# Distributed-Learning-Networking-Group/torchgpipe

Hardware: AMD Instinct MI355X
Metric: U-Net(5,64) GPipe training throughput (samples/sec) (higher is better)
Workload: dtype fp32; 1 GPU; model=U-Net(5,64), experiment=pipeline-1, global_batch=80, input=3x192x192, chunks=2, checkpoint=except_last, parallelism=pp1, transport=none, fused_cells=True, cell_streams=0, overlap_recompute=True, overlap_forward=True, graph_cells=False, hw_queues=4

## Files before the change

torchgpipe_amd/csrc/bindings.cpp:

```cpp
#include <algorithm>
#include <torch/extension.h>
#include <ATen/hip/HIPContext.h>
#include <ATen/hip/impl/HIPGuardImplMasqueradingAsCUDA.h>

#include <vector>

#include "kernels.h"

namespace tgpipe {
namespace {

hipStream_t stream_of(const at::Tensor& t) {
  return at::hip::getCurrentHIPStream(t.device().index()).stream();
}

const int64_t* rng_state(const c10::optional<at::Tensor>& rng, const at::Device& device) {
  if (!rng.has_value() || !rng->defined()) return nullptr;
  TORCH_CHECK(rng->is_cuda() && rng->device() == device && rng->scalar_type() == at::kLong &&
                  rng->is_contiguous() && rng->numel() == 2,
              "rng must be a contiguous int64 [2] (seed, offset) tensor on the op's device");
  return rng->data_ptr<int64_t>();
}

void check_f32_gpu(const at::Tensor& t, const char* name) {
// ... 160 lines not shown
  const int64_t red_channels = flip ? w.size(0) : w.size(1);
  c10::hip::HIPGuardMasqueradingAsCUDA guard(w.device());
  auto u = transform_out(
      out, {wino4_pad_reduction(red_channels), wino4_pad_output(out_channels), 36}, w);
  launch_wino4_weight(w.data_ptr<float>(), u.data_ptr<float>(), out_channels, red_channels, flip,
                      stream_of(w));
  return u;
}

at::Tensor wino4_conv(const at::Tensor& x_in, const at::Tensor& u,
                      const c10::optional<at::Tensor>& bias, int64_t out_channels,
                      int64_t variant, int64_t splits) {
  auto x = x_in.contiguous();
  check_f32_gpu(x, "x");
  check_f32_gpu(u, "u");
  TORCH_CHECK(x.dim() == 4, "x must be NCHW");
  const int64_t n = x.size(0), r = x.size(1), h = x.size(2), w = x.size(3);
  TORCH_CHECK(u.dim() == 3 && u.size(2) == 36 && u.size(0) == wino4_pad_reduction(r) &&
                  u.size(1) == wino4_pad_output(out_channels),
              "F(4x4) transformed weight does not match the input/output channels");
  TORCH_CHECK(u.device() == x.device(), "u must live on the input's device");
  TORCH_CHECK(wino4_supported(n, r, h, w, out_channels),
              "input too large for the F(4x4) kernel (needs < 1 GiB); use wino_conv");
  const float* bptr = nullptr;
  if (bias.has_value() && bias->defined()) {
    check_f32_gpu(*bias, "bias");
    TORCH_CHECK(bias->numel() == out_channels, "bias must have K elements");
    bptr = bias->data_ptr<float>();
  }
  c10::hip::HIPGuardMasqueradingAsCUDA guard(x.device());
  auto y = at::empty({n, out_channels, h, w}, x.options());
  if (y.numel() == 0) return y;
  TORCH_CHECK(variant == -1 || (variant >= 4 && variant <= 15 && variant != 11 && variant != 13) ||
                  variant == 16 || variant == 17 || variant == 18 || (variant >= 20 && variant <= 22),
              "variant must be -1, 4-10, 12, 14-18 or 20-22");
  const WinoPlan plan = wino4_plan(n, r, h, w, out_channels, static_cast<int>(variant),
                                   static_cast<int>(splits));
  at::Tensor ws;
  if (plan.workspace > 0) ws = at::empty({plan.workspace}, x.options());
  launch_wino4_conv(x.data_ptr<float>(), u.data_ptr<float>(), bptr, y.data_ptr<float>(),
                    plan.workspace > 0 ? ws.data_ptr<float>() : nullptr, n, r, h, w,
                    out_channels, plan, stream_of(x));
  return y;
}

at::Tensor wgrad_destination(const c10::optional<at::Tensor>& into, const at::Tensor& x,
                             int64_t k, int64_t c) {
  if (!into.has_value()) return at::empty({k, c, 3, 3}, x.options());
  const at::Tensor& d = *into;
  TORCH_CHECK(d.is_contiguous() && d.scalar_type() == at::kFloat && d.device() == x.device() &&
                  d.dim() == 4 && d.size(0) == k && d.size(1) == c && d.size(2) == 3 &&
                  d.size(3) == 3,
              "into must be a contiguous fp32 [K][C][3][3] tensor on x's device");
  return d;
}

at::Tensor wino_wgrad(const at::Tensor& x_in, const at::Tensor& dy_in, int64_t splits,
                      int64_t variant, const c10::optional<at::Tensor>& into) {
  auto x = x_in.contiguous();
  auto dy = dy_in.contiguous();
  check_f32_gpu(x, "x");
  check_f32_gpu(dy, "dy");
  TORCH_CHECK(x.dim() == 4 && dy.dim() == 4, "x and dy must be NCHW");
  const int64_t n = x.size(0), c = x.size(1), h = x.size(2), w = x.size(3), k = dy.size(1);
  TORCH_CHECK(dy.size(0) == n && dy.size(2) == h && dy.size(3) == w,
              "dy must be [N][K][H][W] of a 3x3/s1/p1 convolution of x");
  TORCH_CHECK(dy.device() == x.device(), "x and dy must share a device");
  TORCH_CHECK(c * h * w < (int64_t{1} << 31) && k * h * w < (int64_t{1} << 31),
// ... 103 lines not shown
  TORCH_CHECK(plan.ksteps * 16 * plan.np < (int64_t{1} << 31) &&
                  plan.mp * plan.np < (int64_t{1} << 31),
              "operands too large for the batched-GEMM kernels");
  float* pm = nullptr;
  int ipg = 0;
  if (stats.has_value() && stats->defined()) {
    check_f32_gpu(*stats, "stats");
    ipg = bg_stats_ipg(n, h, w, static_cast<int>(kind));
    const int64_t groups = (n + ipg - 1) / ipg;
    TORCH_CHECK(stats->device() == x.device() && stats->is_contiguous() &&
                    stats->numel() == 2 * groups * out_channels,
                "stats must be a contiguous [2][ceil(n / bg_stats_ipg)][K] float32 tensor");
    pm = stats->data_ptr<float>();
  }
  auto ws = at::empty({plan.workspace}, x.options());
  launch_bg_conv(x.data_ptr<float>(), a.data_ptr<float>(), bptr, y.data_ptr<float>(),
                 ws.data_ptr<float>(), n, r, h, w, out_channels, plan, stream_of(x), pm,
                 pm == nullptr ? nullptr : pm + stats->numel() / 2, ipg);
  return y;
}

int64_t bg_stats_images(int64_t n, int64_t h, int64_t w, int64_t kind) {
  return bg_stats_ipg(n, h, w, static_cast<int>(kind));
}

int64_t wino4_splits(int64_t n, int64_t c, int64_t k, int64_t h, int64_t w, int64_t variant) {
  if (variant == 0) {
    const int64_t steps = (n * ((h + 3) / 4) * ((w + 3) / 4) + 3) / 4;
    return std::min<int64_t>(wino4_wgrad_splits(n, c, k, h, w), steps);
  }
  return wino4_plan(n, c, h, w, k, static_cast<int>(variant), 0).splits;
}

}
}

TORCH_LIBRARY(tgpipe, m) {
  m.def("dna_forward(Tensor x, float p, float eps, float slope, int seed, int offset, "
        "bool dropout, Tensor? rng=None) -> Tensor[]");
  m.def("dna_backward(Tensor dy, Tensor x, Tensor mean, Tensor rstd, Tensor scale, "
        "float slope) -> Tensor");
  m.def("dropout(Tensor x, float p, int seed, int offset, Tensor? rng=None) -> Tensor");
  m.def("philox_uniform(int n, int seed, int offset, Device device, Tensor? rng=None) -> Tensor");
  m.def("spin(int ns, Device device) -> ()");
  m.def("copy_segments(Tensor[] srcs, Tensor(a!)[] dsts) -> ()");
  m.def("wino_weight(Tensor w, bool flip, Tensor? out=None) -> Tensor");
  m.def("wino_wgrad(Tensor x, Tensor dy, int splits=0, int variant=-1, Tensor? into=None) -> Tensor");
  m.def("wino_conv(Tensor x, Tensor u, Tensor? bias, int out_channels, int variant=-1, "
        "int splits=0) -> Tensor");
  m.def("wino4_weight(Tensor w, bool flip, Tensor? out=None) -> Tensor");
  m.def("wino4_wgrad(Tensor x, Tensor dy, int splits=0, int variant=0, Tensor? into=None) -> Tensor");
  m.def("wino4_conv(Tensor x, Tensor u, Tensor? bias, int out_channels, int variant=-1, "
        "int splits=0) -> Tensor");
  m.def("bg_weight(Tensor w, bool flip, int kind=4, Tensor? out=None, int emu=-1) -> Tensor");
  m.def("wino4_splits(int n, int c, int k, int h, int w, int variant) -> int",
        &tgpipe::wino4_splits);
  m.def("bg_conv(Tensor x, Tensor a, Tensor? bias, int out_channels, int bn=0, int splits=0, "
        "int kind=4, int waves=0, int sub=0, int emu=-1, Tensor(b!)? stats=None) -> Tensor");
  m.def("bg_stats_images(int n, int h, int w, int kind) -> int", &tgpipe::bg_stats_images);
}

TORCH_LIBRARY_IMPL(tgpipe, CUDA, m) {
  m.impl("dna_forward", &tgpipe::dna_forward);
  m.impl("dna_backward", &tgpipe::dna_backward);
  m.impl("dropout", &tgpipe::dropout);
  m.impl("copy_segments", &tgpipe::copy_segments);
  m.impl("wino_weight", &tgpipe::wino_weight);
  m.impl("wino_conv", &tgpipe::wino_conv);
  m.impl("wino_wgrad", &tgpipe::wino_wgrad);
  m.impl("wino4_weight", &tgpipe::wino4_weight);
  m.impl("wino4_conv", &tgpipe::wino4_conv);
  m.impl("wino4_wgrad", &tgpipe::wino4_wgrad);
  m.impl("bg_weight", &tgpipe::bg_weight);
  m.impl("bg_conv", &tgpipe::bg_conv);
}

TORCH_LIBRARY_IMPL(tgpipe, CompositeExplicitAutograd, m) {
  m.impl("philox_uniform", &tgpipe::philox_uniform);
  m.impl("spin", &tgpipe::spin);
}

PYBIND11_MODULE(TORCH_EXTENSION_NAME, m) {
  m.doc() = "torchgpipe_amd native HIP kernels (gfx950)";
}
```

torchgpipe_amd/csrc/kernels.h:

```cpp
#pragma once
#include <hip/hip_runtime.h>
#include <stdint.h>

#include <vector>

namespace tgpipe {

void launch_dna_forward(const float* x, float* y, float* mean, float* rstd, float* scale,
                        int64_t planes, int64_t s, float p, float eps, float slope,
                        uint64_t seed, uint64_t offset, bool dropout, const int64_t* rng,
                        hipStream_t stream);

void launch_dna_backward(const float* dy, const float* x, const float* mean, const float* rstd,
                         const float* scale, float* dx, int64_t planes, int64_t s, float slope,
                         hipStream_t stream);

void launch_dropout(const float* x, float* y, int64_t n, float p, uint64_t seed, uint64_t offset,
                    const int64_t* rng, hipStream_t stream);

void launch_philox_uniform(float* out, int64_t n, uint64_t seed, uint64_t offset,
                           const int64_t* rng, hipStream_t stream);

void launch_spin(uint64_t ns, hipStream_t stream);

struct Segment {
  const void* src;
  void* dst;
  int64_t bytes;
};
constexpr int kMaxSegments = 16;
void launch_segments_copy(const Segment* segs, int count, hipStream_t stream);

int64_t wino_pad_reduction(int64_t r);
int64_t wino_pad_output(int64_t o);
void launch_wino_weight(const float* w, float* u, int64_t out_channels, int64_t red_channels,
                        bool flip, hipStream_t stream);
struct WinoPlan {
  int variant = 0;
  int splits = 1;
  int64_t workspace = 0;
};
WinoPlan wino_plan(int64_t n, int64_t red_channels, int64_t h, int64_t w, int64_t out_channels,
                   int variant, int splits);
void launch_wino_conv(const float* x, const float* u, const float* bias, float* y, float* ws,
                      int64_t n, int64_t red_channels, int64_t h, int64_t w, int64_t out_channels,
                      const WinoPlan& plan, hipStream_t stream);

int64_t wino4_pad_reduction(int64_t r);
int64_t wino4_pad_output(int64_t o);
bool wino4_supported(int64_t n, int64_t r, int64_t h, int64_t w, int64_t o);
void launch_wino4_weight(const float* w, float* u, int64_t out_channels, int64_t red_channels,
                         bool flip, hipStream_t stream);
WinoPlan wino4_plan(int64_t n, int64_t red_channels, int64_t h, int64_t w, int64_t out_channels,
                    int variant, int splits);
void launch_wino4_conv(const float* x, const float* u, const float* bias, float* y, float* ws,
                       int64_t n, int64_t red_channels, int64_t h, int64_t w, int64_t out_channels,
                       const WinoPlan& plan, hipStream_t stream);

struct BgPlan {
  int kind = 4;
  int waves = 8;
  int bn = 64;
  int sub = 1;
  int splits = 1;
  bool emu = false;
  int64_t mp = 0, np = 0, ksteps = 0;
  int64_t workspace = 0;
};
bool bg_emu(int emu);
int bg_pick_bn(int64_t tiles, int kind, bool emu = false);
BgPlan bg_plan(int64_t n, int64_t red_channels, int64_t h, int64_t w, int64_t out_channels,
               int bn, int splits, int kind, int waves, int sub, int emu = -1);
int64_t bg_weight_numel(int64_t out_channels, int64_t red_channels, int kind, int emu = -1);
void launch_bg_weight(const float* w, float* a, int64_t out_channels, int64_t red_channels,
                      bool flip, int kind, hipStream_t stream, int emu = -1);
int bg_stats_ipg(int64_t n, int64_t h, int64_t w, int kind);
void launch_bg_conv(const float* x, const float* a, const float* bias, float* y, float* ws,
                    int64_t n, int64_t red_channels, int64_t h, int64_t w, int64_t out_channels,
                    const BgPlan& plan, hipStream_t stream, float* pm = nullptr,
                    float* pm2 = nullptr, int ipg = 0);


bool wino4_wgrad_supported(int64_t n, int64_t c, int64_t k, int64_t h, int64_t w);
int wino4_wgrad_splits(int64_t n, int64_t c, int64_t k, int64_t h, int64_t w);
int wino4_wgrad_emu_splits(int64_t n, int64_t c, int64_t k, int64_t h, int64_t w);
int64_t wino4_wgrad_emu_workspace(int64_t n, int64_t c, int64_t k, int64_t h, int64_t w,
                                  int splits);
void launch_wino4_wgrad_emu(const float* x, const float* dy, float* dw, float* ws, int64_t n,
                            int64_t c, int64_t k, int64_t h, int64_t w, int splits, bool accum,
                            hipStream_t stream);
// ... 172 lines not shown
```

torchgpipe_amd/csrc/winograd_f4.hip:

```cpp
#include <hip/hip_runtime.h>
#include <stdint.h>

#include <algorithm>
#include <cstdlib>
#include <string>
#include <type_traits>

#include "kernels.h"

namespace tgpipe {
namespace {

typedef float floatx4 __attribute__((ext_vector_type(4)));
typedef float floatx2 __attribute__((ext_vector_type(2)));

constexpr int kP = 36;
constexpr int kC = 4;
constexpr int kOPad = 64;
constexpr int kT = 32;
constexpr int kVImg = kC * kT * kP;

template <int OG>
struct F4Cfg {
  static constexpr int kO = 16 * OG;
  static constexpr int kThreads = 128 * OG;
  static constexpr int kUImg = kC * kO * kP;
  static constexpr int kBuf = kUImg + kVImg;
  static constexpr int kSlabThreads = kThreads - 128;
  static constexpr int kUVec = kUImg / 4 / kSlabThreads;
  static_assert(kUVec * 4 * kSlabThreads == kUImg, "slab waves copy the slab evenly");
};
constexpr uint32_t kBadRow = 0x80000000u;
constexpr uint32_t kBadCol = 0x40000000u;

__device__ __forceinline__ void f4_weight_tile(const float* __restrict__ w, int O, int R, int o,
                                               int r, bool flip, float (&v)[kP]) {
  float g[3][3] = {};
  if (r < R && o < O) {
// ... 209 lines not shown
      acc[4 * q + e] = __builtin_amdgcn_mfma_f32_16x16x4f32(a[q][e], b[q][e], acc[4 * q + e], 0, 0, 0);
  }
  __builtin_amdgcn_sched_group_barrier(0x100, 2 * kAhead, 0);
#pragma unroll
  for (int q = 0; q < kQ; ++q) {
    if (q + kAhead < kQ) __builtin_amdgcn_sched_group_barrier(0x100, 2, 0);
    __builtin_amdgcn_sched_group_barrier(0x008, 4, 0);
  }
}

__device__ __forceinline__ void f4_fwd_offsets(F4Patch& p, int t, int c, int P, int tpi, int TW,
                                               int R, int H, int W) {
  const bool tv = t < P;
  const int tt = tv ? t : 0;
  const int n = tt / tpi;
  const int rem = tt - n * tpi;
  const int ty = rem / TW;
  const int tx = rem - ty * TW;
  const int y0 = 4 * ty - 1, x0 = 4 * tx - 1;
  const int64_t base = (static_cast<int64_t>(n) * R + c) * H * W +
                       static_cast<int64_t>(y0) * W + x0;
#pragma unroll
  for (int i = 0; i < 6; ++i) {
    const bool ok = tv && y0 + i >= 0 && y0 + i < H;
    p.row[i] = ok ? static_cast<uint32_t>((base + static_cast<int64_t>(i) * W) * 4) : kBadRow;
  }
#pragma unroll
  for (int j = 0; j < 6; ++j) {
    const bool ok = x0 + j >= 0 && x0 + j < W;
    p.col[j] = ok ? static_cast<uint32_t>(4 * j) : kBadCol;
  }
}

__device__ __forceinline__ void f4_output_transform(const floatx4 (&acc)[kP],
                                                    float* __restrict__ ydst,
                                                    const float* __restrict__ bias, int tp,
                                                    int tpi, int TW, int H, int W, int O,
                                                    int obase) {
  const int HW = H * W;
  const int pn = tp / tpi;
  const int prem = tp - pn * tpi;
  const int pty = prem / TW;
  const int py = 4 * pty;
  const int px = 4 * (prem - pty * TW);
  const bool full = (W & 3) == 0 && py + 4 <= H;
#pragma unroll
  for (int rp = 0; rp < 2; ++rp) {
    const int o = obase + 2 * rp;
    if (o >= O) continue;
    floatx2 s[4][6];
#pragma unroll
    for (int j = 0; j < 6; ++j) {
      floatx2 m[6];
#pragma unroll
      for (int i = 0; i < 6; ++i) m[i] = floatx2{acc[i * 6 + j][2 * rp], acc[i * 6 + j][2 * rp + 1]};
      const floatx2 a = m[1] + m[2], b = m[1] - m[2], c = m[3] + m[4], d = m[3] - m[4];
      s[0][j] = m[0] + a + c;
      s[1][j] = b + 2.f * d;
      s[2][j] = a + 4.f * c;
      s[3][j] = b + 8.f * d + m[5];
    }
    const floatx2 bv{bias ? bias[o] : 0.f, bias && o + 1 < O ? bias[o + 1] : 0.f};
#pragma unroll
    for (int k = 0; k < 4; ++k) {
      const floatx2 a = s[k][1] + s[k][2], b = s[k][1] - s[k][2];
      const floatx2 c = s[k][3] + s[k][4], d = s[k][3] - s[k][4];
      const floatx2 v0 = s[k][0] + a + c + bv, v1 = b + 2.f * d + bv, v2 = a + 4.f * c + bv;
      const floatx2 v3 = b + 8.f * d + s[k][5] + bv;
#pragma unroll
      for (int e = 0; e < 2; ++e) {
        if (o + e >= O) break;
        float* yp = ydst + (static_cast<int64_t>(pn) * O + o + e) * HW +
                    static_cast<int64_t>(py) * W + px;
        const floatx4 out{v0[e], v1[e], v2[e], v3[e]};
        if (full) {
          *reinterpret_cast<floatx4*>(yp + k * W) = out;
        } else if (py + k < H) {
#pragma unroll
          for (int l = 0; l < 4; ++l)
            if (px + l < W) yp[k * W + l] = out[l];
        }
      }
    }
  }
}

typedef __attribute__((address_space(3))) void lds_void_t;
typedef __attribute__((address_space(1))) void glob_void_t;

template <typename Cfg, int kWaves>
__device__ __forceinline__ void f4_glds_slab(const float* __restrict__ src, float* dst, int sw,
                                             int lane) {
  constexpr int kPieces = Cfg::kUImg / 256;
  static_assert(kPieces % kWaves == 0, "slab waves copy the slab evenly");
#pragma unroll
  for (int i = 0; i < kPieces / kWaves; ++i) {
    const int piece = i * kWaves + sw;
    __builtin_amdgcn_global_load_lds((glob_void_t*)(src + piece * 256 + lane * 4),
                                     (lds_void_t*)(dst + piece * 256), 16, 0, 0);
  }
}

template <int OG, bool kVec, bool kGlds = false, int kAblate = 0>
__global__ __launch_bounds__(F4Cfg<OG>::kThreads, 4 / OG) void f4_conv_kernel(
    const float* __restrict__ x, const float* __restrict__ u, const float* __restrict__ bias,
    float* __restrict__ y, int R, int H, int W, int O, int Rp, int Op, int TH, int TW, int P,
    int tblocks, int oblocks, int splits, uint32_t x_bytes) {
// ... 361 lines not shown
    }
    asm volatile("s_waitcnt lgkmcnt(0)" ::: "memory");
    __builtin_amdgcn_s_barrier();
    auto step = [&](int s, int buf, floatx4 (&cur)[kPer], floatx4 (&nxt)[kPer]) {
      if constexpr (!kDeep && (kDbg & 2) == 0) load_rows(cur, min(s + 3, s_end - 1));
      if (s + 1 < s_end)
        f4_glds_slab<Cfg, kGldsWaves>(ubase + (s + 1) * slab_stride, lds + (buf ^ 1) * kBuf, sw,
                                      lane);
      if constexpr (kDeep && (kDbg & 2) == 0) load_rows(nxt, min(s + 4, s_end - 1));
      __builtin_amdgcn_sched_barrier(0);
      f4_mfma<Cfg>(acc, lds + buf * kBuf, lane, wo, wt);
      __builtin_amdgcn_sched_barrier(0);
      if constexpr ((kDbg & 4) == 0) store_rows(cur, buf ^ 1);
      if constexpr (kDeep) {
        asm volatile("s_waitcnt vmcnt(%0)" ::"n"(kPer) : "memory");
      } else {
        asm volatile("s_waitcnt vmcnt(0)" ::: "memory");
      }
      asm volatile("s_waitcnt lgkmcnt(0)" ::: "memory");
      __builtin_amdgcn_s_barrier();
    };
    floatx4 rodd[kPer];
    int s = s_begin;
    for (; s + 1 < s_end; s += 2) {
      step(s, 0, rreg, rodd);
      step(s + 1, 1, rodd, rreg);
    }
    if (s < s_end) step(s, 0, rreg, rodd);
  }

  const int tp = t0 + wt * 16 + (lane & 15);
  if (tp >= P) return;
  float* ydst = y + static_cast<int64_t>(z) * (P / tpi) * O * HW;
  f4_output_transform(acc, ydst, bias != nullptr && splits == 1 ? bias : nullptr, tp, tpi, TW,
                      H, W, O, o0 + wo * 16 + 4 * (lane >> 4));
}


__global__ __launch_bounds__(256) void f4_input_transform_kernel(
    const float* __restrict__ x, float* __restrict__ v, int R, int H, int W, int TW, int tpi,
    int P, int Rp, int64_t total, uint32_t x_bytes) {
  const int64_t idx = static_cast<int64_t>(blockIdx.x) * blockDim.x + threadIdx.x;
  if (idx >= total) return;
  const int tt = static_cast<int>(idx & 31);
  const int64_t rest = idx >> 5;
  const int c4 = static_cast<int>(rest & 3);
  const int64_t sb = rest >> 2;
  const int steps = Rp / kC;
  const int s = static_cast<int>(sb % steps);
  const int tb = static_cast<int>(sb / steps);
  const int t = tb * kT + tt;
  const int c = s * kC + c4;
  float* dst = v + idx * kP;
  F4Patch p;
  if (t >= P || c >= R) {
#pragma unroll
    for (int q = 0; q < kP / 4; ++q) reinterpret_cast<floatx4*>(dst)[q] = floatx4{0.f, 0.f, 0.f, 0.f};
    return;
  }
  const __amdgpu_buffer_rsrc_t xr =
      __builtin_amdgcn_make_buffer_rsrc(const_cast<float*>(x), static_cast<short>(0),
                                        static_cast<int>(x_bytes), 0x00020000);
  f4_fwd_offsets(p, t, c, P, tpi, TW, R, H, W);
  f4_load_patch<false>(p, xr, 0);
  f4_transform_store(p, dst);
}

template <int OG, int kAhead = 2>
// ... 1616 lines not shown
      }
#pragma unroll
      for (int l = 0; l < TILE; ++l)
        if (l < cols) ts += v[k][l];
    }
    const float tc = static_cast<float>(rows * cols);
    const float tm = ts / tc;
    float tq = 0.f;
#pragma unroll
    for (int k = 0; k < TILE; ++k) {
      if (k >= rows) break;
#pragma unroll
      for (int l = 0; l < TILE; ++l) {
        if (l < cols) {
          const float d = v[k][l] - tm;
          tq += d * d;
        }
      }
    }
    chan_merge_f(cnt, mean, m2, tc, tm, tq);
  }
#pragma unroll
  for (int off = 32; off > 0; off >>= 1) {
    const float nb = __shfl_xor(cnt, off), mb = __shfl_xor(mean, off);
    const float qb = __shfl_xor(m2, off);
    chan_merge_f(cnt, mean, m2, nb, mb, qb);
  }
  if (lane == 0) {
    pm[static_cast<int64_t>(g) * O + o] = mean;
    pm2[static_cast<int64_t>(g) * O + o] = m2;
  }
}

}

int64_t wino4_pad_reduction(int64_t r) { return (r + kC - 1) / kC * kC; }
int64_t wino4_pad_output(int64_t o) { return (o + kOPad - 1) / kOPad * kOPad; }

bool wino4_supported(int64_t n, int64_t r, int64_t h, int64_t w, int64_t o) {
  const int64_t x_bytes = n * r * h * w * 4;
  const int64_t tiles = n * ((h + 3) / 4) * ((w + 3) / 4);
  return x_bytes > 0 && x_bytes < (int64_t{1} << 30) - 64 && tiles < (int64_t{1} << 30) &&
         n * o * h * w < (int64_t{1} << 31) && o < (1 << 24);
}

void launch_wino4_weight(const float* w, float* u, int64_t out_channels, int64_t red_channels,
                         bool flip, hipStream_t stream) {
  const int64_t Op = wino4_pad_output(out_channels);
  const int64_t Rp = wino4_pad_reduction(red_channels);
  const int64_t total = Rp * Op;
  hipLaunchKernelGGL(f4_weight_kernel, dim3(static_cast<unsigned>((total + 255) / 256)), dim3(256),
                     0, stream, w, u, static_cast<int>(out_channels),
                     static_cast<int>(red_channels), static_cast<int>(Op), static_cast<int>(Rp),
                     flip);
}

WinoPlan wino4_plan(int64_t n, int64_t red_channels, int64_t h, int64_t w, int64_t out_channels,
                    int variant, int splits) {
  WinoPlan plan;
  plan.variant = (variant >= 4 && variant <= 12 && variant != 11) || variant == 14 ||
                         variant == 15 || variant == 16 || variant == 17 || variant == 18 ||
                         (variant >= 20 && variant <= 22) ? variant : 5;
  if (plan.variant == 16 && ((w & 3) != 0 || w < 8)) plan.variant = 6;
  if (plan.variant == 17 && ((w & 3) != 0 || w < 24)) plan.variant = 7;
  if (plan.variant >= 20 && plan.variant <= 22 && ((w & 3) != 0 || w < 24)) plan.variant = 6;
  const int og = plan.variant == 5 || plan.variant == 7 || plan.variant == 15 ||
                         plan.variant == 17 ? 2 : 4;
  const int64_t P = n * ((h + 3) / 4) * ((w + 3) / 4);
  const int64_t blocks = ((P + kT - 1) / kT) * ((out_channels + 16 * og - 1) / (16 * og));
  const int64_t steps = wino4_pad_reduction(red_channels) / kC;
  if (splits > 0) {
    plan.splits = static_cast<int>(std::min<int64_t>(splits, steps));
  } else {
    const int64_t cap = og == 4 ? 256 : 512;
    const double step_us = og == 4 ? 2.1 : 1.9;
    const double mb = static_cast<double>(n) * out_channels * h * w * 4 / 1e6;
    int64_t best = 1;
    double best_cost = 0;
    for (int64_t s = 1; s <= std::min<int64_t>(64, steps); ++s) {
      const int64_t rounds = (blocks * s + cap - 1) / cap;
      const double cost = rounds * ((steps + s - 1) / s) * step_us +
                          (s > 1 ? 11.6 + 0.23 * s * mb : 0.0);
      if (s == 1 || cost < best_cost) {
        best = s;
        best_cost = cost;
      }
    }
    plan.splits = static_cast<int>(best);
  }
  plan.workspace = plan.splits > 1 ? plan.splits * n * out_channels * h * w : 0;
  if (plan.variant == 14 || plan.variant == 15) {
    plan.workspace += ((P + kT - 1) / kT) * kT * wino4_pad_reduction(red_channels) * kP;
  }
  return plan;
}

void launch_wino4_conv(const float* x, const float* u, const float* bias, float* y, float* ws,
                       int64_t n, int64_t red_channels, int64_t h, int64_t w, int64_t out_channels,
                       const WinoPlan& plan, hipStream_t stream) {
  const int64_t Rp = wino4_pad_reduction(red_channels);
  const int64_t Op = wino4_pad_output(out_channels);
  const int64_t th = (h + 3) / 4, tw = (w + 3) / 4;
  const int64_t P = n * th * tw;
  const int og = plan.variant == 5 || plan.variant == 7 || plan.variant == 15 ||
                         plan.variant == 17 ? 2 : 4;
  const int tblocks = static_cast<int>((P + kT - 1) / kT);
  if (plan.variant == 18) {
    const int oblocks4 = static_cast<int>((out_channels + 63) / 64);
    const int64_t nwg4 = static_cast<int64_t>(tblocks) * oblocks4 * plan.splits;
    auto kernel = f4_conv_ring_kernel<false>;
    hipLaunchKernelGGL(kernel, dim3(static_cast<unsigned>(nwg4)), dim3(512), 0, stream, x, u,
                       bias, plan.splits > 1 ? ws : y, static_cast<int>(red_channels),
                       static_cast<int>(h), static_cast<int>(w),
                       static_cast<int>(out_channels), static_cast<int>(Rp),
                       static_cast<int>(Op), static_cast<int>(th), static_cast<int>(tw),
                       static_cast<int>(P), tblocks, oblocks4, plan.splits,
                       static_cast<uint32_t>(n * red_channels * h * w * 4));
    if (plan.splits > 1)
      launch_split_reduce(ws, bias, y, n * out_channels * h * w, h * w,
                          static_cast<int>(out_channels), plan.splits, stream);
    return;
  }
// ... 4 lines not shown
    float* vbuf = ws;
    const int64_t vtotal = static_cast<int64_t>(tblocks) * kT * Rp;
    float* split_ws = ws + vtotal * kP;
    hipLaunchKernelGGL(f4_input_transform_kernel, dim3(static_cast<unsigned>((vtotal + 255) / 256)),
                       dim3(256), 0, stream, x, vbuf, static_cast<int>(red_channels),
                       static_cast<int>(h), static_cast<int>(w), static_cast<int>(tw),
                       static_cast<int>(th * tw), static_cast<int>(P), static_cast<int>(Rp),
                       vtotal, static_cast<uint32_t>(n * red_channels * h * w * 4));
    auto gemm = og == 4 ? f4_gemm_kernel<4> : f4_gemm_kernel<2>;
    hipLaunchKernelGGL(gemm, dim3(static_cast<unsigned>(nwg)), dim3(128 * og), 0, stream, vbuf, u,
                       bias, splits > 1 ? split_ws : y, static_cast<int>(h), static_cast<int>(w),
                       static_cast<int>(out_channels), static_cast<int>(Rp), static_cast<int>(Op),
                       static_cast<int>(th), static_cast<int>(tw), static_cast<int>(P), tblocks,
                       oblocks, splits);
    if (splits > 1)
      launch_split_reduce(split_ws, bias, y, n * out_channels * h * w, h * w,
                          static_cast<int>(out_channels), splits, stream);
    return;
  }
  const bool vec = (w & 3) == 0;
  auto kernel = og == 4 ? f4_conv_kernel<4, false>
                        : (vec ? f4_conv_kernel<2, true> : f4_conv_kernel<2, false>);
  if (plan.variant == 6) kernel = f4_conv_kernel<4, false, true>;
  if (plan.variant == 8) kernel = f4_conv_kernel<4, false, true, 1>;
  if (plan.variant == 9) kernel = f4_conv_kernel<4, false, true, 2>;
  if (plan.variant == 10) kernel = f4_conv_kernel<4, false, true, 3>;
  if (plan.variant == 12) kernel = vec ? f4_conv_kernel<4, true, true> : f4_conv_kernel<4, false, true>;
  if (plan.variant == 7) kernel = vec ? f4_conv_kernel<2, true, true> : f4_conv_kernel<2, false, true>;
  if (plan.variant == 16) kernel = tw >= 6 ? f4_conv_rows_kernel<46, 3> : f4_conv_rows_kernel<66, 5>;
  if (plan.variant == 17) kernel = f4_conv_rows_kernel<46, 9, 2>;
  if (plan.variant == 20) kernel = f4_conv_rows_kernel<46, 3, 4, 8>;
  if (plan.variant == 21) kernel = f4_conv_rows_kernel<46, 3, 4, 1>;
  if (plan.variant == 22) kernel = f4_conv_rows_kernel<46, 3, 4, 7>;
  hipLaunchKernelGGL(kernel, dim3(static_cast<unsigned>(nwg)), dim3(128 * og), 0, stream,
                     x, u, bias, splits > 1 ? ws : y, static_cast<int>(red_channels),
                     static_cast<int>(h), static_cast<int>(w), static_cast<int>(out_channels),
                     static_cast<int>(Rp), static_cast<int>(Op), static_cast<int>(th),
                     static_cast<int>(tw), static_cast<int>(P), tblocks, oblocks, splits,
                     static_cast<uint32_t>(n * red_channels * h * w * 4));
  if (splits > 1) {
    launch_split_reduce(ws, bias, y, n * out_channels * h * w, h * w,
                        static_cast<int>(out_channels), splits, stream);
  }
}

bool wino4_wgrad_supported(int64_t n, int64_t c, int64_t k, int64_t h, int64_t w) {
  const int64_t lim = (int64_t{1} << 30) - 64;
  const int64_t tiles = n * ((h + 3) / 4) * ((w + 3) / 4);
  return n * c * h * w * 4 < lim && n * k * h * w * 4 < lim && n * c * h * w > 0 &&
         n * k * h * w > 0 && tiles + 64 < (int64_t{1} << 30);
}

int wino4_wgrad_splits(int64_t n, int64_t c, int64_t k, int64_t h, int64_t w) {
  const int64_t blocks = ((c + 31) / 32) * ((k + 63) / 64);
  const int64_t steps = (n * ((h + 3) / 4) * ((w + 3) / 4) + 3) / 4;
  const double mb = static_cast<double>(((c + 31) / 32) * 32) * (((k + 63) / 64) * 64) * 9 * 4 /
                    1e6;
  int best = 1;
  double best_cost = 0;
  for (int64_t s = 1; s <= std::min<int64_t>(512, steps); ++s) {
    const int64_t rounds = (blocks * s + 255) / 256;
    const double cost = rounds * ((steps + s - 1) / s) * 2.5 + (s > 1 ? 5.0 + 0.8 * s * mb : 0.0);
    if (s == 1 || cost < best_cost) {
      best = static_cast<int>(s);
      best_cost = cost;
    }
  }
// ... 341 lines not shown
```

torchgpipe_amd/ops/conv.py:

```python
import os
import threading
from typing import Any, Dict, List, Optional, Sequence, Tuple
import weakref

import torch
from torch import Tensor, nn
import torch.nn.functional as F

from torchgpipe_amd.ops import _ext, gradacc

__all__ = ['WinogradConv2d', 'winograd_conv2d', 'wino_eligible', 'new_step',
           'clear_winograd_caches', 'cache_bytes', 'refresh_step_caches', 'hold_cache',
           'size_cache_budget', 'conv_with_bn_stats']

_STEP = 0
_CACHE_BYTES: Dict[torch.device, int] = {}
_BUDGET: Optional[int] = None
_DEVICE_BUDGET: Dict[torch.device, int] = {}
_FRACTION = os.environ.get('TGPIPE_WINOGRAD_CACHE_FRACTION')
CACHE_PEAK_FRACTION: Optional[float] = float(_FRACTION) if _FRACTION else None
PRESPLIT_MB = max(0, int(os.environ.get('TGPIPE_CG_PRESPLIT_MB', '2048')))


def new_step() -> None:
# ... 181 lines not shown
    hit = _SCANS.get(module)
    if hit is None or hit[0] != _CACHE_EPOCH:
        refs = [weakref.ref(v) for m in module.modules() for v in list(vars(m).values())
                if isinstance(v, (_TransformCache, _GroupCache))]
        hit = _SCANS[module] = (_CACHE_EPOCH, refs)
    return [v for v in (r() for r in hit[1]) if v is not None]


def refresh_step_caches(module: nn.Module) -> None:
    sources: List[Tensor] = []
    for v in _step_caches(module):
        v.refresh()
        if isinstance(v, _TransformCache):
            sources += v.derived()
        else:
            sources += [t for t in (v.cat, v.cat_t) if t is not None]
    if _ext._loaded:
        sources += [p for p in module.parameters() if p.is_cuda]
        if sources:
            torch.ops.tgpipe.conv_gemm_presplit_refresh(sources)


def clear_winograd_caches(module: torch.nn.Module) -> None:
    for m in module.modules():
        for attr in ('_wino', '_wt_cache'):
            cache = getattr(m, attr, None)
            if isinstance(cache, _TransformCache):
                cache.clear()


F4_MIN_PLANE = 8
_F4_FUSED_VARIANT = int(os.environ.get('TGPIPE_F4_FUSED_VARIANT', '16'))
F4_ROWS_MIN_WIDTH = 24
F4_MAX_BYTES = (1 << 30) - 64


F4_MIN_PLANE_WIDE = 6
F4_WIDE_CHANNELS = 512


F4_MAX_CACHE_BYTES = 2 << 30
F4_ENABLED = os.environ.get('TGPIPE_WINOGRAD_F4', '1') != '0'


def _use_f4(x: Tensor, out_channels: int = 0) -> bool:
    if not F4_ENABLED or x.shape[1] * out_channels * 36 * 4 > F4_MAX_CACHE_BYTES:
        return False
    plane = min(x.shape[2], x.shape[3])
    wide = (plane >= F4_MIN_PLANE_WIDE and out_channels >= F4_WIDE_CHANNELS
            and x.shape[1] >= F4_WIDE_CHANNELS and x.shape[0] <= 24)
    return (plane >= F4_MIN_PLANE or wide) and x.numel() * x.element_size() < F4_MAX_BYTES


BG_ENABLED = os.environ.get('TGPIPE_WINOGRAD_BG', '1') != '0'
BG_MIN_CHANNELS = int(os.environ.get('TGPIPE_WINOGRAD_BG_MIN_CHANNELS', '256'))


def _bg_kind(x: Tensor, out_channels: int) -> int:
    r = x.shape[1]
    plane = min(x.shape[2], x.shape[3])
    if not BG_ENABLED or r < BG_MIN_CHANNELS or out_channels < BG_MIN_CHANNELS or plane < 6:
        return 0
    kind = 2 if plane < 8 else 4
    positions = 16 if kind == 2 else 36
    if r * out_channels * positions * 4 > F4_MAX_CACHE_BYTES or \
            x.numel() * x.element_size() >= F4_MAX_BYTES:
        return 0
    tiles = x.shape[0] * -(-x.shape[2] // kind) * -(-x.shape[3] // kind)
    if positions * max(r, out_channels) * (tiles + 192) >= (1 << 31):
        return 0
    return kind


def _conv(x: Tensor, cache: _TransformCache, weight: Tensor, bias: Optional[Tensor],
          flip: bool) -> Tensor:
    ops = _ext.require(x)
    out_channels = weight.shape[1] if flip else weight.shape[0]
    kind = _bg_kind(x, out_channels)
    if kind:
        return ops.bg_conv(x, cache.get(weight, flip, bg=kind), bias, out_channels, 0, 0, kind)
    if _use_f4(x, out_channels):
        tiles = x.shape[0] * ((x.shape[2] + 3) // 4) * ((x.shape[3] + 3) // 4)
        blocks = -(-tiles // 32) * -(-out_channels // 64)
        if out_channels >= 512:
            small = blocks < 160 or min(x.shape[2], x.shape[3]) < F4_MIN_PLANE
            variant = 15 if small else 14
        else:
            variant = 7 if out_channels <= 32 or blocks < 160 else _F4_FUSED_VARIANT
            if variant == 16 and x.shape[3] < F4_ROWS_MIN_WIDTH:
                variant = 6
        return ops.wino4_conv(x, cache.get(weight, flip, True), bias, out_channels, variant)
    return ops.wino_conv(x, cache.get(weight, flip), bias, out_channels)


class _WinogradConv(torch.autograd.Function):
    @staticmethod
    def forward(ctx, x: Tensor, weight: Tensor, bias: Optional[Tensor],
                cache: _TransformCache) -> Tensor:
        y = _conv(x.contiguous(), cache, weight, bias, False)
        ctx.save_for_backward(x, weight)
        ctx.cache = cache
        ctx.has_bias = bias is not None
        ctx.param = weight
        return y

    @staticmethod
    def backward(ctx, dy: Tensor):
        x, weight = ctx.saved_tensors
        dy = dy.contiguous()
        dx, dw = _conv_grads(x, weight, dy, ctx.cache, ctx.needs_input_grad[0],
                             ctx.needs_input_grad[1], ctx.param)
        ctx.param = None
        db = None
        if ctx.has_bias and ctx.needs_input_grad[2]:
            db = dy.sum((0, 2, 3))
        return dx, dw, db, None


class _WinogradConvStats(torch.autograd.Function):

    @staticmethod
    def forward(ctx, x: Tensor, weight: Tensor, cache: _TransformCache,
                kind: int) -> Tuple[Tensor, Tensor]:
# ... 155 lines not shown
```

Before: 723.0 samples/sec.

## Add persistent F(4x4) Winograd conv kernel that pipelines across work items

```diff
diff --git a/torchgpipe_amd/csrc/bindings.cpp b/torchgpipe_amd/csrc/bindings.cpp
--- a/torchgpipe_amd/csrc/bindings.cpp
+++ b/torchgpipe_amd/csrc/bindings.cpp
@@ -216,8 +216,8 @@
   auto y = at::empty({n, out_channels, h, w}, x.options());
   if (y.numel() == 0) return y;
   TORCH_CHECK(variant == -1 || (variant >= 4 && variant <= 15 && variant != 11 && variant != 13) ||
-                  variant == 16 || variant == 17 || variant == 18 || (variant >= 20 && variant <= 22),
-              "variant must be -1, 4-10, 12, 14-18 or 20-22");
+                  variant == 16 || variant == 17 || variant == 18 || (variant >= 20 && variant <= 26),
+              "variant must be -1, 4-10, 12, 14-18 or 20-26");
   const WinoPlan plan = wino4_plan(n, r, h, w, out_channels, static_cast<int>(variant),
                                    static_cast<int>(splits));
   at::Tensor ws;
@@ -387,6 +387,17 @@
   return wino4_plan(n, c, h, w, k, static_cast<int>(variant), 0).splits;
 }
 
+int64_t wino4_persist_grid_op(int64_t wgs) {
+  return wino4_persist_grid(static_cast<int>(std::min<int64_t>(wgs, 1 << 20)));
+}
+
+std::vector<int64_t> wino4_persist_items_op(int64_t nwg, int64_t grid, int64_t bid) {
+  TORCH_CHECK(nwg > 0 && grid > 0 && grid <= nwg && bid >= 0 && bid < grid &&
+                  nwg < (int64_t{1} << 30),
+              "wino4_persist_items: needs 0 <= bid < grid <= nwg < 2^30");
+  return wino4_persist_items(nwg, grid, bid);
+}
+
 }
 }
 
@@ -410,6 +421,9 @@
   m.def("bg_weight(Tensor w, bool flip, int kind=4, Tensor? out=None, int emu=-1) -> Tensor");
   m.def("wino4_splits(int n, int c, int k, int h, int w, int variant) -> int",
         &tgpipe::wino4_splits);
+  m.def("wino4_persist_grid(int wgs=-1) -> int", &tgpipe::wino4_persist_grid_op);
+  m.def("wino4_persist_items(int nwg, int grid, int bid) -> int[]",
+        &tgpipe::wino4_persist_items_op);
   m.def("bg_conv(Tensor x, Tensor a, Tensor? bias, int out_channels, int bn=0, int splits=0, "
         "int kind=4, int waves=0, int sub=0, int emu=-1, Tensor(b!)? stats=None) -> Tensor");
   m.def("bg_stats_images(int n, int h, int w, int kind) -> int", &tgpipe::bg_stats_images);
diff --git a/torchgpipe_amd/csrc/kernels.h b/torchgpipe_amd/csrc/kernels.h
--- a/torchgpipe_amd/csrc/kernels.h
+++ b/torchgpipe_amd/csrc/kernels.h
@@ -56,6 +56,8 @@
 void launch_wino4_conv(const float* x, const float* u, const float* bias, float* y, float* ws,
                        int64_t n, int64_t red_channels, int64_t h, int64_t w, int64_t out_channels,
                        const WinoPlan& plan, hipStream_t stream);
+int wino4_persist_grid(int wgs);
+std::vector<int64_t> wino4_persist_items(int64_t nwg, int64_t grid, int64_t bid);
 
 struct BgPlan {
   int kind = 4;
diff --git a/torchgpipe_amd/csrc/winograd_f4.hip b/torchgpipe_amd/csrc/winograd_f4.hip
--- a/torchgpipe_amd/csrc/winograd_f4.hip
+++ b/torchgpipe_amd/csrc/winograd_f4.hip
@@ -2,8 +2,11 @@
 #include <stdint.h>
 
 #include <algorithm>
+#include <atomic>
 #include <cstdlib>
+#include <stdexcept>
 #include <string>
+#include <vector>
 #include <type_traits>
 
 #include "kernels.h"
@@ -279,11 +282,12 @@
   }
 }
 
+template <bool kStore = true, bool kEarlyBias = false>
 __device__ __forceinline__ void f4_output_transform(const floatx4 (&acc)[kP],
                                                     float* __restrict__ ydst,
                                                     const float* __restrict__ bias, int tp,
                                                     int tpi, int TW, int H, int W, int O,
-                                                    int obase) {
+                                                    int obase, float* sink = nullptr) {
   const int HW = H * W;
   const int pn = tp / tpi;
   const int prem = tp - pn * tpi;
@@ -291,10 +295,17 @@
   const int py = 4 * pty;
   const int px = 4 * (prem - pty * TW);
   const bool full = (W & 3) == 0 && py + 4 <= H;
+  float early[4] = {0.f, 0.f, 0.f, 0.f};
 #pragma unroll
   for (int rp = 0; rp < 2; ++rp) {
     const int o = obase + 2 * rp;
     if (o >= O) continue;
+    if constexpr (kEarlyBias) {
+      if (rp == 0 && bias != nullptr) {
+#pragma unroll
+        for (int e = 0; e < 4; ++e) early[e] = bias[min(obase + e, O - 1)];
+      }
+    }
     floatx2 s[4][6];
 #pragma unroll
     for (int j = 0; j < 6; ++j) {
@@ -307,7 +318,17 @@
       s[2][j] = a + 4.f * c;
       s[3][j] = b + 8.f * d + m[5];
     }
-    const floatx2 bv{bias ? bias[o] : 0.f, bias && o + 1 < O ? bias[o + 1] : 0.f};
+    if constexpr (kEarlyBias) {
+      if (rp == 0) {
+        __builtin_amdgcn_sched_barrier(0);
+        asm volatile("" : "+v"(early[0]), "+v"(early[1]), "+v"(early[2]), "+v"(early[3]));
+#pragma unroll
+        for (int e = 0; e < 4; ++e) early[e] = obase + e < O ? early[e] : 0.f;
+      }
+    }
+    const floatx2 bv = kEarlyBias
+                           ? floatx2{early[2 * rp], early[2 * rp + 1]}
+                           : floatx2{bias ? bias[o] : 0.f, bias && o + 1 < O ? bias[o + 1] : 0.f};
 #pragma unroll
     for (int k = 0; k < 4; ++k) {
       const floatx2 a = s[k][1] + s[k][2], b = s[k][1] - s[k][2];
@@ -320,6 +341,10 @@
         float* yp = ydst + (static_cast<int64_t>(pn) * O + o + e) * HW +
                     static_cast<int64_t>(py) * W + px;
         const floatx4 out{v0[e], v1[e], v2[e], v3[e]};
+        if constexpr (!kStore) {
+          *sink += (out[0] + out[1]) + (out[2] + out[3]);
+          continue;
+        }
         if (full) {
           *reinterpret_cast<floatx4*>(yp + k * W) = out;
         } else if (py + k < H) {
@@ -747,8 +772,283 @@
   const int tp = t0 + wt * 16 + (lane & 15);
   if (tp >= P) return;
   float* ydst = y + static_cast<int64_t>(z) * (P / tpi) * O * HW;
+  if constexpr ((kDbg & 48) != 0) {
+    int none = 0;
+    asm volatile("" : "+s"(none));
+    if constexpr ((kDbg & 32) != 0) {
+      if (tp >= none) return;
+    }
+    float sink = 0.f;
+    f4_output_transform<false>(acc, ydst, bias != nullptr && splits == 1 ? bias : nullptr, tp,
+                               tpi, TW, H, W, O, o0 + wo * 16 + 4 * (lane >> 4), &sink);
+    if (tp < none) ydst[tp] = sink;
+    return;
+  }
   f4_output_transform(acc, ydst, bias != nullptr && splits == 1 ? bias : nullptr, tp, tpi, TW,
                       H, W, O, o0 + wo * 16 + 4 * (lane >> 4));
+}
+
+struct F4Sched {
+  int first, stride, end;
+};
+__host__ __device__ inline F4Sched f4_persist_sched(int nwg, int grid, int bid) {
+  const int ng = grid < 8 ? grid : 8;
+  const int xcd = bid % ng;
+  const int qq = nwg / ng, rr = nwg % ng;
+  const int start = xcd < rr ? xcd * (qq + 1) : rr * (qq + 1) + (xcd - rr) * qq;
+  const int len = qq + (xcd < rr ? 1 : 0);
+  const int stride = (grid - xcd + ng - 1) / ng;
+  return F4Sched{start + bid / ng, stride, start + len};
+}
+
+struct F4Item {
+  int t0, o0, z, s0, n, n0;
+};
+constexpr int kPersistMinSteps = 5;
+
+template <int kDbg = 0>
+__global__ __launch_bounds__(512, 1) void f4_conv_persist_kernel(
+    const float* __restrict__ x, const float* __restrict__ u, const float* __restrict__ bias,
+    float* __restrict__ y, int R, int H, int W, int O, int Rp, int Op, int TH, int TW, int P,
+    int tblocks, int oblocks, int splits, uint32_t x_bytes) {
+  constexpr int OG = 4, kRS = 46, kPer = 3;
+  using Cfg = F4Cfg<OG>;
+  using Rows = F4Rows<kRS>;
+  constexpr int kO = Cfg::kO;
+  constexpr int kBuf = Cfg::kBuf;
+  constexpr int kSlot = Rows::kSlot;
+  __shared__ float lds[2 * kBuf + 2 * kSlot];
+  float* const raw = lds + 2 * kBuf;
+
+  const int nwg = tblocks * oblocks * splits;
+  const F4Sched sched = f4_persist_sched(nwg, gridDim.x, blockIdx.x);
+
+  const int tid = threadIdx.x;
+  const int lane = tid & 63;
+  const int wave = tid >> 6;
+  const int wo = wave % OG;
+  const int wt = wave / OG;
+  const int HW = H * W;
+  const int tpi = TH * TW;
+  const int nsteps = Rp / kC;
+  const uint32_t step_bytes = static_cast<uint32_t>(kC) * HW * 4;
+
+  auto item = [&](int wgid) __attribute__((always_inline)) {
+    F4Item it;
+    const int ob = wgid % oblocks;
+    const int tb = (wgid / oblocks) % tblocks;
+    it.z = wgid / (oblocks * tblocks);
+    it.t0 = tb * kT;
+    it.o0 = ob * kO;
+    it.s0 = it.z * nsteps / splits;
+    it.n = (it.z + 1) * nsteps / splits - it.s0;
+    it.n0 = min(TW - (it.t0 % tpi) % TW, kT);
+    return it;
+  };
+
+  floatx4 acc[kP];
+#pragma unroll
+  for (int i = 0; i < kP; ++i) acc[i] = floatx4{0.f, 0.f, 0.f, 0.f};
+  const float* bz = bias != nullptr && splits == 1 ? bias : nullptr;
+  auto finish = [&](const F4Item& it) __attribute__((always_inline)) {
+    const int tp = it.t0 + wt * 16 + (lane & 15);
+    float* ydst = y + static_cast<int64_t>(it.z) * (P / tpi) * O * HW;
+    const int obase = it.o0 + wo * 16 + 4 * (lane >> 4);
+    if constexpr ((kDbg & 16) != 0) {
+      int none = 0;
+      asm volatile("" : "+s"(none));
+      if (tp < P) {
+        float sink = 0.f;
+        f4_output_transform<false, true>(acc, ydst, bz, tp, tpi, TW, H, W, O, obase, &sink);
+        if (tp < none) ydst[tp] = sink;
+      }
+    } else {
+      if (tp < P)
+        f4_output_transform<true, true>(acc, ydst, bz, tp, tpi, TW, H, W, O, obase);
+    }
+#pragma unroll
+    for (int i = 0; i < kP; ++i) acc[i] = floatx4{0.f, 0.f, 0.f, 0.f};
+  };
+
+  const __amdgpu_buffer_rsrc_t xr =
+      __builtin_amdgcn_make_buffer_rsrc(const_cast<float*>(x), static_cast<short>(0),
+                                        static_cast<int>(x_bytes), 0x00020000);
+  F4Item a = item(sched.first);
+  F4Item b = a;
+  int next = sched.first + sched.stride;
+  bool more = next < sched.end;
+  int r = 0;
+
+  if (wave < 2) {
+    const int tl = wave * 16 + (lane & 15);
+    float* vmine = lds + Cfg::kUImg + ((lane >> 4) * kT + tl) * kP;
+    auto rows_at = [&](int n0) -> const float* {
+      const int seg = tl < n0 ? 0 : 1 + (tl - n0) / TW;
+      return raw + ((lane >> 4) * Rows::kCS + tl + 2 * seg) * 4;
+    };
+    F4Patch p;
+    f4_fwd_offsets(p, a.t0 + tl, lane >> 4, P, tpi, TW, R, H, W);
+    F4Patch first = p;
+    f4_load_patch<false>(first, xr, a.s0 * step_bytes);
+    f4_load_patch<false>(p, xr, (a.s0 + 1) * step_bytes);
+    f4_transform_store(first, vmine);
+    asm volatile("s_waitcnt lgkmcnt(0)" ::: "memory");
+    __builtin_amdgcn_s_barrier();
+    auto read_rows = [&](const float* rp) {
+#pragma unroll
+      for (int i = 0; i < 6; ++i) {
+        p.d[i * 6 + 0] = rp[i * kRS * 4 + 3];
+        const floatx4 mid = *reinterpret_cast<const floatx4*>(rp + i * kRS * 4 + 4);
+#pragma unroll
+        for (int j = 0; j < 4; ++j) p.d[i * 6 + 1 + j] = mid[j];
+        p.d[i * 6 + 5] = rp[i * kRS * 4 + 8];
+      }
+    };
+    const float* rcur = rows_at(a.n0);
+    const float* rnxt = rcur;
+    int buf = 0;
+    for (;;) {
+      f4_transform_store(p, vmine + (buf ^ 1) * kBuf);
+      __builtin_amdgcn_sched_barrier(0);
+      if (r == a.n) {
+        finish(a);
+        if (!more) break;
+        a = b;
+        rcur = rnxt;
+        r = 0;
+        next += sched.stride;
+        more = next < sched.end;
+      }
+      read_rows((r + 2 < a.n ? rcur : rnxt) + buf * kSlot);
+      __builtin_amdgcn_sched_barrier(0);
+      if (r == 0 && more) {
+        b = item(next);
+        rnxt = rows_at(b.n0);
+      }
+      f4_mfma<Cfg>(acc, lds + buf * kBuf, lane, wo, wt);
+      asm volatile("s_waitcnt lgkmcnt(0)" ::: "memory");
+      __builtin_amdgcn_s_barrier();
+      buf ^= 1;
+      ++r;
+    }
+  } else {
+    const int stid = tid - 128;
+    const int sw = stid >> 6;
+    constexpr int kGldsWaves = Cfg::kSlabThreads / 64;
+    const int64_t slab_stride = static_cast<int64_t>(Op / 16) * (kC * 16 * kP);
+    auto rows_of = [&](const F4Item& it, uint32_t (&xoff)[kPer],
+                       int (&slot)[kPer]) __attribute__((always_inline)) {
+      const int nseg = it.n0 < kT ? 1 + (kT - it.n0 + TW - 1) / TW : 1;
+      const int rs = kT + 2 * nseg;
+#pragma unroll
+      for (int k = 0; k < kPer; ++k) {
+        const int e = (stid + k * Cfg::kSlabThreads) % (kC * 6 * rs);
+        const int c = e / (6 * rs);
+        const int er = e - c * 6 * rs;
+        const int i = er / rs;
+        const int q = er - i * rs;
+        int g;
+        const int ck = f4_rows_segment(q, it.n0, TW, &g);
+        const int tf = g == 0 ? it.t0 : it.t0 + it.n0 + (g - 1) * TW;
+        const int n = tf / tpi;
+        const int rem = tf - n * tpi;
+        const int ty = rem / TW;
+        const int yy = 4 * ty - 1 + i;
+        const int xx = 4 * (rem - ty * TW - 1 + ck);
+        const bool ok = tf < P && yy >= 0 && yy < H && xx >= 0 && xx < W;
+        const int64_t idx = (static_cast<int64_t>(n) * R + c) * HW + static_cast<int64_t>(yy) * W + xx;
+        xoff[k] = ok ? static_cast<uint32_t>(idx * 4) : kBadRow;
+        slot[k] = (c * Rows::kCS + i * kRS + q) * 4;
+      }
+    };
+    static_assert(kPer * Cfg::kSlabThreads >= kC * 6 * kRS, "every chunk has a lane");
+    auto slab_of = [&](const F4Item& it) {
+      return u + static_cast<int64_t>(it.o0 / 16) * (kC * 16 * kP) + it.s0 * slab_stride;
+    };
+    auto load_rows = [&](floatx4 (&rreg)[kPer], const uint32_t (&xoff)[kPer], int s) {
+#pragma unroll
+      for (int k = 0; k < kPer; ++k) {
+        const auto v = __builtin_amdgcn_raw_buffer_load_b128(xr, xoff[k] + s * step_bytes, 0, 0);
+        rreg[k] = floatx4{__uint_as_float(v[0]), __uint_as_float(v[1]), __uint_as_float(v[2]),
+                          __uint_as_float(v[3])};
+      }
+    };
+    const uint32_t raw_lds = static_cast<uint32_t>(reinterpret_cast<uintptr_t>((lds_void_t*)raw));
+    auto store_rows = [&](const floatx4 (&rreg)[kPer], const int (&slot)[kPer], int slot_index) {
+#pragma unroll
+      for (int k = 0; k < kPer; ++k) {
+        const uint32_t ad = raw_lds + (slot_index * kSlot + slot[k]) * 4;
+        asm volatile("ds_write_b128 %0, %1" ::"v"(ad), "v"(rreg[k]) : "memory");
+      }
+    };
+    uint32_t xa[kPer], xb[kPer];
+    int sa[kPer], sb[kPer];
+    rows_of(a, xa, sa);
+#pragma unroll
+    for (int k = 0; k < kPer; ++k) {
+      xb[k] = xa[k];
+      sb[k] = sa[k];
+    }
+    const float* ua = slab_of(a);
+    const float* ub = ua;
+    floatx4 rreg[kPer], rodd[kPer];
+    load_rows(rreg, xa, a.s0 + 2);
+    f4_glds_slab<Cfg, kGldsWaves>(ua, lds, sw, lane);
+    store_rows(rreg, sa, 0);
+    __builtin_amdgcn_sched_barrier(0);
+    load_rows(rreg, xa, a.s0 + 3);
+    asm volatile("s_waitcnt vmcnt(%0)" ::"n"(kPer) : "memory");
+    asm volatile("s_waitcnt lgkmcnt(0)" ::: "memory");
+    __builtin_amdgcn_s_barrier();
+    auto step = [&](int buf, floatx4 (&cur)[kPer],
+                    floatx4 (&nxt)[kPer]) __attribute__((always_inline)) {
+      const bool n1 = r + 1 >= a.n, n3 = r + 3 >= a.n, n4 = r + 4 >= a.n;
+      if (!n1 || more)
+        f4_glds_slab<Cfg, kGldsWaves>(n1 ? ub : ua + (r + 1) * slab_stride, lds + (buf ^ 1) * kBuf,
+                                      sw, lane);
+      uint32_t x4[kPer];
+#pragma unroll
+      for (int k = 0; k < kPer; ++k) x4[k] = n4 ? xb[k] : xa[k];
+      load_rows(nxt, x4, n4 ? b.s0 + (r + 4 - a.n) : a.s0 + r + 4);
+      __builtin_amdgcn_sched_barrier(0);
+      if (r == 0 && more) {
+        b = item(next);
+        rows_of(b, xb, sb);
+        ub = slab_of(b);
+      }
+      __builtin_amdgcn_sched_barrier(0);
+      f4_mfma<Cfg>(acc, lds + buf * kBuf, lane, wo, wt);
+      __builtin_amdgcn_sched_barrier(0);
+      int s3[kPer];
+#pragma unroll
+      for (int k = 0; k < kPer; ++k) s3[k] = n3 ? sb[k] : sa[k];
+      store_rows(cur, s3, buf ^ 1);
+      asm volatile("s_waitcnt vmcnt(%0)" ::"n"(kPer) : "memory");
+      asm volatile("s_waitcnt lgkmcnt(0)" ::: "memory");
+      __builtin_amdgcn_s_barrier();
+    };
+    auto boundary = [&]() __attribute__((always_inline)) {
+      finish(a);
+      if (!more) return false;
+      a = b;
+      ua = ub;
+#pragma unroll
+      for (int k = 0; k < kPer; ++k) {
+        xa[k] = xb[k];
+        sa[k] = sb[k];
+      }
+      r = 0;
+      next += sched.stride;
+      more = next < sched.end;
+      return true;
+    };
+    for (;;) {
+      step(0, rreg, rodd);
+      if (++r == a.n && !boundary()) break;
+      step(1, rodd, rreg);
+      if (++r == a.n && !boundary()) break;
+    }
+  }
 }
 
 
@@ -2431,6 +2731,37 @@
   }
 }
 
+std::atomic<int> persist_grid{0};
+
+int device_cus() {
+  static std::atomic<int> cus[64];
+  int dev = 0;
+  if (hipGetDevice(&dev) != hipSuccess || dev < 0 || dev >= 64) return 256;
+  int n = cus[dev].load();
+  if (n == 0) {
+    if (hipDeviceGetAttribute(&n, hipDeviceAttributeMultiprocessorCount, dev) != hipSuccess ||
+        n <= 0)
+      n = 256;
+    cus[dev].store(n);
+  }
+  return n;
+}
+
+}
+
+int wino4_persist_grid(int wgs) {
+  if (wgs < 0) return persist_grid.load();
+  return persist_grid.exchange(wgs);
+}
+
+std::vector<int64_t> wino4_persist_items(int64_t nwg, int64_t grid, int64_t bid) {
+  if (nwg <= 0 || grid <= 0 || grid > nwg || bid < 0 || bid >= grid || nwg >= (int64_t{1} << 30))
+    throw std::runtime_error("wino4_persist_items: needs 0 <= bid < grid <= nwg < 2^30");
+  const F4Sched s = f4_persist_sched(static_cast<int>(nwg), static_cast<int>(grid),
+                                     static_cast<int>(bid));
+  std::vector<int64_t> items;
+  for (int i = s.first; i < s.end; i += s.stride) items.push_back(i);
+  return items;
 }
 
 int64_t wino4_pad_reduction(int64_t r) { return (r + kC - 1) / kC * kC; }
@@ -2459,10 +2790,14 @@
   WinoPlan plan;
   plan.variant = (variant >= 4 && variant <= 12 && variant != 11) || variant == 14 ||
                          variant == 15 || variant == 16 || variant == 17 || variant == 18 ||
-                         (variant >= 20 && variant <= 22) ? variant : 5;
+                         (variant >= 20 && variant <= 26) ? variant : 5;
+  const bool persist = plan.variant == 23 || plan.variant == 26;
+  if (persist && ((w & 3) != 0 || w < 24)) plan.variant = 16;
   if (plan.variant == 16 && ((w & 3) != 0 || w < 8)) plan.variant = 6;
   if (plan.variant == 17 && ((w & 3) != 0 || w < 24)) plan.variant = 7;
-  if (plan.variant >= 20 && plan.variant <= 22 && ((w & 3) != 0 || w < 24)) plan.variant = 6;
+  if ((plan.variant >= 20 && plan.variant <= 22) || plan.variant == 24 || plan.variant == 25) {
+    if ((w & 3) != 0 || w < 24) plan.variant = 6;
+  }
   const int og = plan.variant == 5 || plan.variant == 7 || plan.variant == 15 ||
                          plan.variant == 17 ? 2 : 4;
   const int64_t P = n * ((h + 3) / 4) * ((w + 3) / 4);
@@ -2487,6 +2822,8 @@
     }
     plan.splits = static_cast<int>(best);
   }
+  if ((plan.variant == 23 || plan.variant == 26) && steps / plan.splits < kPersistMinSteps)
+    plan.variant = 16;
   plan.workspace = plan.splits > 1 ? plan.splits * n * out_channels * h * w : 0;
   if (plan.variant == 14 || plan.variant == 15) {
     plan.workspace += ((P + kT - 1) / kT) * kT * wino4_pad_reduction(red_channels) * kP;
@@ -2557,7 +2894,15 @@
   if (plan.variant == 20) kernel = f4_conv_rows_kernel<46, 3, 4, 8>;
   if (plan.variant == 21) kernel = f4_conv_rows_kernel<46, 3, 4, 1>;
   if (plan.variant == 22) kernel = f4_conv_rows_kernel<46, 3, 4, 7>;
-  hipLaunchKernelGGL(kernel, dim3(static_cast<unsigned>(nwg)), dim3(128 * og), 0, stream,
+  if (plan.variant == 24) kernel = f4_conv_rows_kernel<46, 3, 4, 16>;
+  if (plan.variant == 25) kernel = f4_conv_rows_kernel<46, 3, 4, 32>;
+  int64_t grid = nwg;
+  if (plan.variant == 23 || plan.variant == 26) {
+    kernel = plan.variant == 23 ? f4_conv_persist_kernel<0> : f4_conv_persist_kernel<16>;
+    const int forced = persist_grid.load();
+    grid = std::min<int64_t>(nwg, forced > 0 ? forced : device_cus());
+  }
+  hipLaunchKernelGGL(kernel, dim3(static_cast<unsigned>(grid)), dim3(128 * og), 0, stream,
                      x, u, bias, splits > 1 ? ws : y, static_cast<int>(red_channels),
                      static_cast<int>(h), static_cast<int>(w), static_cast<int>(out_channels),
                      static_cast<int>(Rp), static_cast<int>(Op), static_cast<int>(th),
diff --git a/torchgpipe_amd/ops/conv.py b/torchgpipe_amd/ops/conv.py
--- a/torchgpipe_amd/ops/conv.py
+++ b/torchgpipe_amd/ops/conv.py
@@ -237,6 +237,10 @@
 F4_MIN_PLANE = 8
 _F4_FUSED_VARIANT = int(os.environ.get('TGPIPE_F4_FUSED_VARIANT', '16'))
 F4_ROWS_MIN_WIDTH = 24
+F4_PERSIST = os.environ.get('TGPIPE_F4_PERSIST', '1') != '0'
+F4_PERSIST_MIN_WIDTH = 192
+F4_PERSIST_MAX_CHANNELS = 128
+F4_PERSIST_MIN_BLOCKS = 512
 F4_MAX_BYTES = (1 << 30) - 64
 
 
@@ -294,6 +298,10 @@
             variant = 7 if out_channels <= 32 or blocks < 160 else _F4_FUSED_VARIANT
             if variant == 16 and x.shape[3] < F4_ROWS_MIN_WIDTH:
                 variant = 6
+            elif (variant == 16 and F4_PERSIST and x.shape[3] >= F4_PERSIST_MIN_WIDTH
+                  and x.shape[3] % 4 == 0 and x.shape[1] <= F4_PERSIST_MAX_CHANNELS
+                  and blocks >= F4_PERSIST_MIN_BLOCKS):
+                variant = 23
         return ops.wino4_conv(x, cache.get(weight, flip, True), bias, out_channels, variant)
     return ops.wino_conv(x, cache.get(weight, flip), bias, out_channels)
 
```

After: 725.4 samples/sec (median of 6 runs). About the same (+0.3%).
